# shenyunhang/APE

Measured on AMD Instinct MI355X. Metric: images/sec @1024^2 APE-L_D fwd, higher is better.
Workload: dtype bf16

## Files before the change

### ape_amd/_lib.py

```python
import ctypes
import os
from ctypes import POINTER, Structure, c_char_p, c_double, c_float, c_int, c_int32, c_int64, c_void_p

_HERE = os.path.dirname(os.path.abspath(__file__))
LIB_PATH = os.path.join(_HERE, "lib", "libape_hip.so")

DT_F32 = 0
DT_BF16 = 1
DT_F16 = 2
ACT_NONE, ACT_RELU, ACT_GELU, ACT_SWIGLU, ACT_SILU = 0, 1, 2, 3, 4
MASK_NONE, MASK_ZERO_INPUT, MASK_ZERO_OUTPUT = 0, 1, 2


class GemmArgs(Structure):
    _fields_ = [
        ("A", c_void_p), ("W", c_void_p), ("C", c_void_p), ("bias", c_void_p), ("residual", c_void_p),
        ("rowmask", c_void_p), ("rope_cos", c_void_p), ("rope_sin", c_void_p),
        ("M", c_int32), ("N", c_int32), ("K", c_int32),
        ("lda", c_int32), ("ldw", c_int32), ("ldc", c_int32), ("ldr", c_int32),
        ("in_dt", c_int32), ("out_dt", c_int32), ("res_dt", c_int32),
        ("act", c_int32), ("mask_mode", c_int32), ("trans_out", c_int32),
        ("rope_rows", c_int32), ("rope_hd", c_int32), ("rope_cols", c_int32), ("vec_ok", c_int32),
        ("alpha", c_float), ("clamp", c_float),
        ("splitk", c_int32), ("tile64", c_int32), ("workspace", c_void_p),
# ... 36 lines not shown
    "ape_hip_stuff_collapse": (c_int, [c_void_p, c_int, c_int, c_int, c_int, c_void_p, c_int, c_void_p]),
    "ape_hip_sem_class_weights": (c_int, [c_void_p, c_int, c_void_p, c_void_p, c_int, c_int, c_int, c_float, c_void_p, c_int, c_int, c_void_p]),
    "ape_hip_pan_class_scores": (c_int, [c_void_p, c_int, c_void_p, c_void_p, c_int, c_int, c_float, c_int, c_float, c_void_p, c_void_p,
                                         c_void_p, c_void_p, c_void_p]),
    "ape_hip_argmax_labels": (c_int, [c_void_p, ctypes.c_size_t, c_int, ctypes.c_size_t, c_float, c_void_p, c_void_p]),
    "ape_hip_sdma_usable": (c_int, [c_void_p, c_void_p]),
    "ape_hip_sdma_d2h": (c_int, [c_void_p, c_void_p, ctypes.c_size_t]),
    "ape_hip_sdma_d2h_multi": (c_int, [c_int, ctypes.POINTER(c_void_p), ctypes.POINTER(c_void_p), ctypes.POINTER(ctypes.c_size_t), c_int]),
    "ape_hip_sdma_engines": (c_int, [c_void_p, c_void_p]),
    "ape_hip_row_stats": (c_int, [c_void_p, c_int, c_int, c_int, c_int, c_float, c_void_p, c_void_p, c_void_p]),
    "ape_hip_gemv": (c_int, [c_void_p, c_int, c_void_p, c_int, c_int, c_void_p, c_void_p, c_int, c_int, c_int, c_int,
                             c_float, c_void_p]),
    "ape_hip_gemv_affine": (c_int, [c_void_p, c_int, c_void_p, c_int, c_int, c_void_p, c_void_p, c_int, c_int, c_int, c_int,
                                    c_float, c_void_p, c_void_p, c_int, c_void_p, c_int, c_void_p]),
    "ape_hip_layernorm": (c_int, [POINTER(LayerNormArgs), c_void_p]),
    "ape_hip_postnorm_residual": (c_int, [c_void_p, c_int, c_int, c_void_p, c_void_p, c_float, c_void_p, c_int, c_void_p, c_int, c_int,
                                          c_int, c_int, c_void_p]),
    "ape_hip_groupnorm_workspace_floats": (c_int, [c_int, c_int]),
    "ape_hip_groupnorm": (c_int, [POINTER(GroupNormArgs), c_void_p]),
    "ape_hip_ms_deform_attn_forward": (c_int, [c_void_p, c_int, POINTER(c_int64), POINTER(c_int64), c_void_p, c_void_p,
                                               c_void_p, c_int, c_int, c_int, c_int, c_int, c_int, c_void_p]),
    "ape_hip_msda_fused": (c_int, [c_void_p, c_int, c_int, POINTER(c_int64), POINTER(c_int64), c_void_p, c_int, c_void_p,
                                   c_int, c_void_p, c_int, c_int, c_int, c_int, c_int, c_int, c_void_p]),
    "ape_hip_msda_fused_h": (c_int, [c_void_p, c_int, c_int, POINTER(c_int64), POINTER(c_int64), c_void_p, c_int, c_void_p,
                                     c_int, c_void_p, c_int, c_int, c_int, c_int, c_int, c_int, c_void_p]),
    "ape_hip_attention": (c_int, [c_void_p, c_int, c_void_p, c_int, c_void_p, c_int, c_void_p, c_int, c_int, c_int, c_int,
                                  c_int, c_float, c_int, c_void_p]),
    "ape_hip_geometry": (c_int, [c_int, c_int, c_int, c_int, POINTER(c_int), c_void_p, c_int, c_void_p, c_float, c_float, c_float,
                                 c_void_p, c_int, c_void_p, c_void_p, c_void_p, c_void_p, c_void_p, c_void_p, c_void_p, c_void_p,
                                 c_void_p]),
# ... 5 lines not shown
                                         c_int, c_int, c_float, c_int, c_void_p]),
    "ape_hip_embed_tokens": (c_int, [c_void_p, c_int, c_void_p, c_int, c_void_p, c_int, c_int, c_void_p, c_int, c_int, c_int, c_int,
                                     c_int, c_int, c_void_p]),
    "ape_hip_patchify": (c_int, [c_void_p, c_int, c_int, c_void_p, c_int, c_int, POINTER(c_float), POINTER(c_float), c_void_p,
                                 c_int, c_int, c_void_p]),
    "ape_hip_im2col3x3": (c_int, [c_void_p, c_int, c_void_p, c_int, c_int, c_int, c_void_p, c_int, c_int, c_void_p]),
    "ape_hip_maxpool2x2": (c_int, [c_void_p, c_int, c_void_p, c_int, c_int, c_int, c_void_p, c_int, c_int, c_void_p]),
    "ape_hip_gather_rows": (c_int, [c_void_p, c_int, c_void_p, c_int, c_int, c_void_p, c_int, c_int, c_void_p]),
    "ape_hip_gather_rows_i64": (c_int, [c_void_p, c_int, c_void_p, c_int, c_int, c_void_p, c_int, c_int, c_void_p]),
    "ape_hip_nms_mask_words": (c_int, [c_int]),
    "ape_hip_nms_mask": (c_int, [c_void_p, c_void_p, c_int, c_float, c_void_p, c_void_p]),
    "ape_hip_nms_scan_segments": (c_int, [c_void_p, c_int, c_void_p, c_int, c_int, c_void_p, c_void_p, c_void_p]),
    "ape_hip_nms_scan_classes": (c_int, [c_void_p, c_int, c_void_p, c_int, c_void_p, c_void_p, c_void_p]),
    "ape_hip_vl_pool_workspace_floats": (c_int, [c_int, c_int]),
    "ape_hip_vl_pool": (c_int, [c_void_p, c_int, c_void_p, c_int, c_int, c_int, c_int, c_void_p, c_void_p, c_void_p, c_void_p]),
    "ape_hip_segment_softmax": (c_int, [c_void_p, c_int, c_int, c_int, c_int, c_void_p, c_void_p, c_int, c_int, c_void_p]),
    "ape_hip_colstats_workspace_floats": (c_int, [c_int, c_int]),
    "ape_hip_colstats": (c_int, [c_void_p, c_int, c_int, c_int, c_void_p, c_void_p, c_void_p, c_void_p, c_void_p]),
    "ape_hip_transpose": (c_int, [c_void_p, c_int, c_int, c_int, c_int, c_void_p, c_void_p, c_void_p, c_void_p, c_int, c_int,
                                  c_void_p]),
    "ape_hip_mask_upsample_bits": (c_int, [c_void_p, c_int, c_int, c_int, c_int, c_int, c_int, c_void_p, c_void_p]),
    "ape_hip_roi_align_bits": (c_int, [c_void_p, c_int, c_int, c_void_p, c_int, c_int, c_void_p, c_void_p]),
    "ape_hip_paste_bits": (c_int, [c_void_p, c_int, c_void_p, c_int, c_int, c_int, c_void_p, c_void_p]),
    "ape_hip_mask_upsample_sigmoid": (c_int, [c_void_p, c_int, c_int, c_int, c_int, c_int, c_int, c_int, c_int, c_void_p, c_int, c_int,
                                              c_void_p]),
    "ape_hip_box_refine": (c_int, [c_void_p, c_int, c_void_p, c_void_p, c_int, c_int, c_float, c_void_p, c_void_p, c_void_p]),
    "ape_hip_det_records": (c_int, [c_void_p, c_void_p, c_void_p, c_void_p, c_void_p, c_int, c_void_p, c_void_p, c_void_p, c_void_p]),
    "ape_hip_query_init": (c_int, [c_void_p, c_void_p, c_int, c_void_p, c_int, c_float, c_int, c_void_p, c_void_p, c_int, c_int, c_void_p,
                                   c_void_p]),
    "ape_hip_query_finish": (c_int, [c_void_p, c_int, c_void_p, c_int, c_int, c_int, c_void_p, c_void_p, c_float, c_void_p, c_void_p,
# ... 81 lines not shown
```

### ape_amd/csrc/norm.hip

```cpp
#include "common.h"
#include "../../include/ape_hip.h"

__device__ __forceinline__ float ln_act(float x, int act) {
  if (act == APE_ACT_RELU) return fmaxf(x, 0.f);
  if (act == APE_ACT_GELU) return 0.5f * x * (1.f + erff(x * 0.70710678118654752440f));
  return x;
}

template <typename TX, typename TY, typename TA, int NV4>
__global__ __launch_bounds__(256) void layernorm_kernel(const ApeLayerNormArgs p) {
  const int lane = threadIdx.x & 63;
  const int row = blockIdx.x * 4 + (threadIdx.x >> 6);
  if (row >= p.M) return;
  const TX* x = reinterpret_cast<const TX*>(p.x) + (size_t)row * p.ldx;
  TY* y = reinterpret_cast<TY*>(p.y) + (size_t)row * p.ldy;
  const TA* add = p.add ? reinterpret_cast<const TA*>(p.add) + (size_t)row * p.ldadd : nullptr;
  TY* y2 = p.y2 ? reinterpret_cast<TY*>(p.y2) + (size_t)row * p.ldy2 : nullptr;
  const int C = p.C;
  const float invC = 1.f / (float)C;
  float v[NV4][4];
  float s = 0.f;
#pragma unroll
  for (int i = 0; i < NV4; ++i) {
    const int c = (i * 64 + lane) * 4;
    if (c + 3 < C) {
      ld4<TX>(x + c, v[i]);
    } else {
#pragma unroll
      for (int r = 0; r < 4; ++r) v[i][r] = (c + r < C) ? ldf<TX>(x + c + r) : 0.f;
    }
    s += (v[i][0] + v[i][1]) + (v[i][2] + v[i][3]);
  }
  const float mean = wave_sum(s) * invC;
  float q = 0.f;
#pragma unroll
  for (int i = 0; i < NV4; ++i) {
    const int c = (i * 64 + lane) * 4;
#pragma unroll
    for (int r = 0; r < 4; ++r) {
      const float d = (c + r < C) ? v[i][r] - mean : 0.f;
      q = fmaf(d, d, q);
    }
  }
  const float rstd = rsqrtf(wave_sum(q) * invC + p.eps);
#pragma unroll
  for (int i = 0; i < NV4; ++i) {
    const int c = (i * 64 + lane) * 4;
    if (c >= p.Cpad) continue;
    float o[4], o2[4];
    if (c + 3 < C) {
      float w4[4], b4[4];
      ld4<float>(p.w + c, w4);
      ld4<float>(p.b + c, b4);
#pragma unroll
      for (int r = 0; r < 4; ++r) o[r] = ln_act((v[i][r] - mean) * rstd * w4[r] + b4[r], p.act);
      st4<TY>(y + c, o);
      if (y2 != nullptr) {
        ld4<TA>(add + c, o2);
#pragma unroll
        for (int r = 0; r < 4; ++r) o2[r] += o[r];
        st4<TY>(y2 + c, o2);
      }
      continue;
    }
#pragma unroll
    for (int r = 0; r < 4; ++r) {
      if (c + r < C) {
        o[r] = ln_act((v[i][r] - mean) * rstd * p.w[c + r] + p.b[c + r], p.act);
        o2[r] = (y2 != nullptr) ? o[r] + ldf<TA>(add + c + r) : 0.f;
      } else {
        o[r] = 0.f; o2[r] = 0.f;
      }
    }
    if (c + 3 < p.Cpad) {
      st4<TY>(y + c, o);
      if (y2 != nullptr) st4<TY>(y2 + c, o2);
    } else {
      for (int r = 0; r < 4 && c + r < p.Cpad; ++r) { stf<TY>(y + c + r, o[r]); if (y2 != nullptr) stf<TY>(y2 + c + r, o2[r]); }
    }
  }
  for (int c = NV4 * 256 + lane; c < p.Cpad; c += 64) { stf<TY>(y + c, 0.f); if (y2 != nullptr) stf<TY>(y2 + c, 0.f); }
}

template <typename TX, typename TY, typename TA>
__global__ __launch_bounds__(256) void layernorm_generic_kernel(const ApeLayerNormArgs p) {
  const int lane = threadIdx.x & 63;
  const int row = blockIdx.x * 4 + (threadIdx.x >> 6);
  if (row >= p.M) return;
  const TX* x = reinterpret_cast<const TX*>(p.x) + (size_t)row * p.ldx;
  TY* y = reinterpret_cast<TY*>(p.y) + (size_t)row * p.ldy;
  const TA* add = p.add ? reinterpret_cast<const TA*>(p.add) + (size_t)row * p.ldadd : nullptr;
  TY* y2 = p.y2 ? reinterpret_cast<TY*>(p.y2) + (size_t)row * p.ldy2 : nullptr;
  const int C = p.C;
  const float invC = 1.f / (float)C;
  float s = 0.f;
  for (int c = lane; c < C; c += 64) s += ldf<TX>(x + c);
// ... 366 lines not shown
```

### ape_amd/csrc/vlpool.hip

```cpp
#include "common.h"
#include "../../include/ape_hip.h"

#define VL_CHUNK 128
#define VL_H 8

__global__ __launch_bounds__(256) void vl_smax_partial_kernel(const float* __restrict__ S, int lds, int T, float* __restrict__ pmax) {
  __shared__ float sh[256];
  const int t = threadIdx.x, h = t & 7;
  const int base = blockIdx.x * VL_CHUNK;
  float m = -INFINITY;
  for (int k = 0; k < VL_CHUNK / 32; ++k) {
    const int tok = base + k * 32 + (t >> 3);
    if (tok < T) m = fmaxf(m, S[(size_t)tok * lds + h]);
  }
  sh[t] = m;
  __syncthreads();
  if (t < VL_H) {
    float a = -INFINITY;
    for (int j = t; j < 256; j += 8) a = fmaxf(a, sh[j]);
    pmax[blockIdx.x * VL_H + t] = a;
  }
}

template <typename TX>
// ... 46 lines not shown
  }
  for (int c = t; c < C; c += 256) {
    float acc[VL_H];
#pragma unroll
    for (int h = 0; h < VL_H; ++h) acc[h] = 0.f;
    for (int r = 0; r < cnt; ++r) {
      const float xv = ldf<TX>(x + (size_t)(base + r) * ldx + c);
#pragma unroll
      for (int h = 0; h < VL_H; ++h) acc[h] = fmaf(P[r][h], xv, acc[h]);
    }
#pragma unroll
    for (int h = 0; h < VL_H; ++h) pacc[((size_t)blockIdx.x * VL_H + h) * C + c] = acc[h];
  }
}

__global__ __launch_bounds__(256) void vl_pool_final_kernel(const float* __restrict__ pacc, const float* __restrict__ psum, int nchunk,
                                                            int C, const float* __restrict__ sub, float* __restrict__ out) {
  __shared__ float sa[8][32];
  __shared__ float sl[256];
  const int h = blockIdx.x, t = threadIdx.x;
  const int kg = t >> 5, cl = t & 31;
  const int c = blockIdx.y * 32 + cl;
  float l = 0.f;
  for (int k = t; k < nchunk; k += 256) l += psum[k * VL_H + h];
  sl[t] = l;
  float a = 0.f;
  if (c < C) for (int k = kg; k < nchunk; k += 8) a += pacc[((size_t)k * VL_H + h) * C + c];
  sa[kg][cl] = a;
  __syncthreads();
  for (int o = 128; o > 0; o >>= 1) { if (t < o) sl[t] += sl[t + o]; __syncthreads(); }
  if (t < 32 && c < C) {
    float acc = 0.f;
#pragma unroll
    for (int g = 0; g < 8; ++g) acc += sa[g][t];
    out[h * C + c] = acc / sl[0] - (sub != nullptr ? sub[c] : 0.f);
  }
}

extern "C" int ape_hip_vl_pool_workspace_floats(int T, int C) {
  const int nchunk = ceil_div(T, VL_CHUNK);
  return nchunk * VL_H * (C + 2);
}

extern "C" int ape_hip_vl_pool(const float* S, int lds, const void* x, int ldx, int x_dt, int T, int C, float* workspace,
                               const float* sub, float* out, void* stream) {
  APE_CHECK_ARG(S && x && workspace && out && T > 0 && C > 0, "ape_hip_vl_pool: bad args");
  const int nchunk = ceil_div(T, VL_CHUNK);
  float* pmax = workspace;
  float* psum = pmax + nchunk * VL_H;
  float* pacc = psum + nchunk * VL_H;
  hipStream_t s = (hipStream_t)stream;
  APE_LAUNCH(vl_smax_partial_kernel, dim3(nchunk), dim3(256), 0, s, S, lds, T, pmax);
  if (x_dt == APE_DT_F16) APE_LAUNCH(vl_pool_partial_kernel<f16_t>, dim3(nchunk), dim3(256), 0, s, S, lds, (const f16_t*)x, ldx, T, C, pmax, nchunk, pacc, psum);
  else if (x_dt == APE_DT_BF16) APE_LAUNCH(vl_pool_partial_kernel<bf16_t>, dim3(nchunk), dim3(256), 0, s, S, lds, (const bf16_t*)x, ldx, T, C, pmax, nchunk, pacc, psum);
  else
    APE_LAUNCH(vl_pool_partial_kernel<float>, dim3(nchunk), dim3(256), 0, s, S, lds, (const float*)x, ldx, T, C, pmax, nchunk, pacc, psum);
  APE_LAUNCH(vl_pool_final_kernel, dim3(VL_H, ceil_div(C, 32)), dim3(256), 0, s, pacc, psum, nchunk, C, sub, out);
  APE_CHECK_LAUNCH("ape_hip_vl_pool");
  return 0;
}


template <typename TC>
__global__ __launch_bounds__(256) void head_gemv_kernel(const float* __restrict__ x, int ldx, const float* __restrict__ W,
                                                        const float* __restrict__ bias, float* __restrict__ out, int ldo, int H,
                                                        int N, int D, float alpha, TC* __restrict__ out_bf16, int ldob) {
  const int lane = threadIdx.x & 63;
  const int row = blockIdx.x * 4 + (threadIdx.x >> 6);
  if (row >= H * N) return;
  const int h = row / N, n = row % N;
  const float* w = W + (size_t)row * D;
  const float* xr = x + (size_t)h * ldx;
  float s = 0.f;
// ... 31 lines not shown
```

### ape_amd/layers/fuse_helper.py

```python
import torch
import torch.nn as nn

from .. import ops
from ..packing import attach_cache, f32, ln_params, pack_matrix


class BiMultiHeadAttention(nn.Module):
    def __init__(self, v_dim, l_dim, embed_dim, num_heads, dropout=0.1, stable_softmax_2d=False,
                 clamp_min_for_underflow=True, clamp_max_for_overflow=True, use_attention_mask_v=False):
        super().__init__()
        self.embed_dim, self.num_heads, self.head_dim = embed_dim, num_heads, embed_dim // num_heads
        self.v_dim, self.l_dim = v_dim, l_dim
        assert self.head_dim * num_heads == embed_dim
        self.scale = self.head_dim ** (-0.5)
        self.dropout = dropout
        self.v_proj = nn.Linear(v_dim, embed_dim)
        self.l_proj = nn.Linear(l_dim, embed_dim)
        self.values_v_proj = nn.Linear(v_dim, embed_dim)
        self.values_l_proj = nn.Linear(l_dim, embed_dim)
        self.out_v_proj = nn.Linear(embed_dim, v_dim)
        self.out_l_proj = nn.Linear(embed_dim, l_dim)
        self.stable_softmax_2d = stable_softmax_2d
        self.clamp_min_for_underflow = clamp_min_for_underflow
        self.clamp_max_for_overflow = clamp_max_for_overflow
# ... 84 lines not shown
    def forward_tokens(self, x, lvl_pos, l, dt, defer_language=False):
        if l.shape[0] == 1:
            v_new, qp, ljob = self.forward_tokens_single(x, lvl_pos, l, dt)
        else:
            v_new, qp, l_new = self.forward_tokens_dense(x, lvl_pos, l, dt)
            ljob = ops._Joined(l_new)
        return (v_new, qp, ljob) if defer_language else (v_new, qp, ljob.join())

    def forward_tokens_single(self, x, lvl_pos, l, dt):
        P = self.packed(dt)
        a = self.attn
        l_n = ops.layernorm(l, P["lnl"][0], P["lnl"][1], P["lnl"][2], out_dtype=torch.float32)
        k = ops.gemv(l_n, P["wl"], P["bl"])
        vl = ops.gemv(l_n, P["wvl"], P["bvl"])
        gdv, lnb = ops.gemv(vl, P["wov"], P["bov"], scale=P["gv"], add=P["lnv"][1][None, :])
        v_new, qp = ops.layernorm(x, P["lnv"][0], lnb[0], P["lnv"][2], out_dtype=dt, add=lvl_pos)

        def language_side():
            kh = k.view(a.num_heads, a.head_dim)
            u, u_c = ops.head_gemv(kh, P["wvT"], bf16_copy=dt if dt in ops.HALF16 else True)
            c = ops.head_gemv(kh, P["bv1"], alpha=a.scale)
            _, sbias = ops.gemv(gdv, u, alpha=-a.scale, add=c.view(1, -1))
            S = ops.gemm(v_new, u_c if dt in ops.HALF16 else u, sbias[0], alpha=a.scale, out_dtype=torch.float32)
            pooled = ops.vl_pool(S, v_new, gdv[0])
            ol = ops.head_gemv(pooled, P["wvv"], P["bvv"])
            return ops.gemv(ol.view(1, -1), P["wol"], P["bol"], scale=P["gl"], add=l_n)[1]

        return v_new, qp, ops.fork(language_side)

    def forward(self, v, l, attention_mask_v=None, attention_mask_l=None):
        if attention_mask_l is not None:
            raise NotImplementedError("ape_amd BiAttentionBlock: per-token language masks (un-reduced expression tokens, "
                                      "text_feature_reduce_before_fusion=False) are not implemented")
        dt = getattr(self, "compute_dtype", torch.bfloat16)
        vs, ls = [], []
        for b in range(v.shape[0]):
            zeros = torch.zeros_like(v[b], dtype=dt)
            vn, _, ln = self.forward_tokens(v[b].to(dt).contiguous(), zeros, l[b].float().contiguous(), dt)
            vs.append(vn.to(v.dtype))
# ... 3 lines not shown
```

### ape_amd/ops.py

```python
import ctypes
import math
import os

import numpy as np
import torch

from . import _lib
from ._lib import (ACT_GELU, ACT_NONE, ACT_RELU, ACT_SILU, ACT_SWIGLU, DT_BF16, DT_F32, MASK_NONE,
                   MASK_ZERO_INPUT, MASK_ZERO_OUTPUT)

_DT = {torch.float32: DT_F32, torch.bfloat16: DT_BF16, torch.float16: _lib.DT_F16}
HALF16 = (torch.bfloat16, torch.float16)


def _dt(t):
    try:
        return _DT[t.dtype]
    except KeyError:
        raise TypeError(f"ape_amd: unsupported dtype {t.dtype} (float32 / bfloat16 / float16 only)")


def _dev(*ts):
    for t in ts:
        if t is not None and not t.is_cuda:
# ... 232 lines not shown
        out = torch.empty((M, cpad), dtype=odt, device=x.device)
    args = _lib.LayerNormArgs()
    args.x, args.w, args.b, args.y = x.data_ptr(), _f32vec(w, "w").data_ptr(), _f32vec(b, "b").data_ptr(), out.data_ptr()
    args.M, args.C, args.Cpad = M, C, cpad
    args.ldx, args.ldy = _ld(x), _ld(out)
    args.x_dt, args.y_dt, args.act, args.eps = _dt(x), _dt(out), act, float(eps)
    if add is not None:
        _rowmajor(add, "add")
        if out2 is None:
            out2 = torch.empty((M, cpad), dtype=out.dtype, device=x.device)
        args.add, args.y2, args.ldadd, args.ldy2, args.add_dt = add.data_ptr(), out2.data_ptr(), _ld(add), _ld(out2), _dt(add)
    _lib.check(_lib.load().ape_hip_layernorm(ctypes.byref(args), _stream()), "ape_hip_layernorm")
    return (out, out2) if add is not None else out


def postnorm_residual(stream, t, norm, copy_dtype=None):
    _dev(stream, t)
    _rowmajor(stream, "stream")
    if stream.dtype != torch.float32:
        raise TypeError("ape_amd.ops.postnorm_residual: the residual stream is float32")
    M, C = stream.shape
    if copy_dtype not in (None, torch.float32) + HALF16 or (t is not None and t.dtype not in (torch.float32,) + HALF16):
        raise TypeError("ape_amd.ops.postnorm_residual: t and the copy are float32, bfloat16 or float16")
    copy = torch.empty((M, C), dtype=copy_dtype, device=stream.device) if copy_dtype is not None else None
    w = b = None
    eps = 0.0
    if t is not None:
        _rowmajor(t, "t")
        if tuple(t.shape) != (M, C):
            raise ValueError("ape_amd.ops.postnorm_residual: t must match the stream")
# ... 282 lines not shown


def vl_pool(scores, x, sub=None):
    _dev(scores, x, sub)
    _rowmajor(scores, "scores"), _rowmajor(x, "x")
    if scores.dtype != torch.float32 or scores.shape[1] != 8:
        raise ValueError("ape_amd.ops.vl_pool: scores must be float32 [T,8]")
    T, C = x.shape
    if sub is not None and sub.numel() != C:
        raise ValueError("ape_amd.ops.vl_pool: sub must have one entry per channel")
    lib = _lib.load()
    ws = torch.empty((lib.ape_hip_vl_pool_workspace_floats(T, C),), dtype=torch.float32, device=x.device)
    out = torch.empty((8, C), dtype=torch.float32, device=x.device)
    rc = lib.ape_hip_vl_pool(_p(scores), _ld(scores), _p(x), _ld(x), _dt(x), T, C, _p(ws), _p(_f32vec(sub, "sub")), _p(out), _stream())
    _lib.check(rc, "ape_hip_vl_pool")
    return out


def segment_softmax(scores, nseg, gmax, out_dtype):
    _dev(scores, gmax)
    _rowmajor(scores, "scores")
    if scores.dtype != torch.float32 or gmax.dtype != torch.float32 or scores.shape[1] % nseg:
        raise ValueError("ape_amd.ops.segment_softmax: scores must be float32 [T, nseg*L], gmax a float32 scalar")
    T, C = scores.shape
    out = torch.empty((T, C), dtype=out_dtype, device=scores.device)
    rc = _lib.load().ape_hip_segment_softmax(_p(scores), _ld(scores), T, nseg, C // nseg, _p(gmax), _p(out), _ld(out), _dt(out),
                                             _stream())
    _lib.check(rc, "ape_hip_segment_softmax")
    return out

# ... 962 lines not shown
```

### include/ape_hip.h

```cpp
#ifndef APE_HIP_H
#define APE_HIP_H
#include <stdint.h>

#ifdef __cplusplus
extern "C" {
#endif

#define APE_DT_F32 0
#define APE_DT_BF16 1
#define APE_DT_F16 2

#define APE_ACT_NONE 0
#define APE_ACT_RELU 1
#define APE_ACT_GELU 2
#define APE_ACT_SWIGLU 3
#define APE_ACT_SILU 4

#define APE_MASK_NONE 0
#define APE_MASK_ZERO_INPUT 1
#define APE_MASK_ZERO_OUTPUT 2

const char* ape_hip_last_error(void);
int ape_hip_abi_version(void);
int ape_hip_sizeof_args(int which);
// ... 57 lines not shown

typedef struct ApeLayerNormArgs {
  const void* x;
  const float* w;
  const float* b;
  void* y;
  const void* add;
  void* y2;
  int32_t M, C, Cpad;
  int32_t ldx, ldy, ldadd, ldy2;
  int32_t x_dt, y_dt, add_dt;
  int32_t act;
  float eps;
} ApeLayerNormArgs;
int ape_hip_layernorm(const ApeLayerNormArgs* args, void* stream);

int ape_hip_postnorm_residual(const void* t, int ldt, int t_dt, const float* w, const float* b, float eps, float* stream, int lds,
                              void* copy, int ldc, int copy_dt, int M, int C, void* hip_stream);


typedef struct ApeGroupNormArgs {
  const void* x;
  const float* w;
  const float* b;
  void* y;
  const void* add;
  float* workspace;
  int32_t HW, C, G;
  int32_t ldx, ldy, ldadd;
  int32_t x_dt, y_dt, add_dt;
// ... 27 lines not shown
int ape_hip_im2col3x3(const void* x, int ldx, const int32_t* perm, int H, int W, int C, void* out, int ldo, int dt, void* stream);
int ape_hip_maxpool2x2(const void* x, int ldx, const int32_t* perm, int H, int W, int C, void* out, int ldo, int dt, void* stream);
int ape_hip_gather_rows(const void* x, int ldx, const int32_t* idx, int n, int C, void* out, int ldo, int dt, void* stream);
int ape_hip_gather_rows_i64(const void* x, int ldx, const int64_t* idx, int n, int C, void* out, int ldo, int dt, void* stream);

int ape_hip_nms_mask_words(int n);
int ape_hip_nms_mask(const float* boxes_xyxy, const int32_t* groups, int n, float iou_thr, uint64_t* mask, void* stream);
int ape_hip_nms_scan_segments(const uint64_t* mask, int n, const int32_t* seg_offsets, int num_segments, int max_segment,
                              const uint8_t* valid, uint8_t* keep, void* stream);
int ape_hip_nms_scan_classes(const uint64_t* mask, int n, const int32_t* order, int num_classes, const uint8_t* valid,
                             uint8_t* keep, void* stream);

int ape_hip_vl_pool_workspace_floats(int T, int C);
int ape_hip_vl_pool(const float* S, int lds, const void* x, int ldx, int x_dt, int T, int C, float* workspace, const float* sub,
                    float* out, void* stream);
int ape_hip_head_gemv(const float* x, int ldx, const float* W, const float* bias, float* out, int ldo, int H, int N, int D,
                      float alpha, void* out_bf16, int ldob, int copy_dt, void* stream);

int ape_hip_segment_softmax(const float* S, int lds, int T, int nseg, int L, const float* gmax, void* out, int ldo, int out_dt,
                            void* stream);
int ape_hip_colstats_workspace_floats(int T, int C);
int ape_hip_colstats(const float* S, int lds, int T, int C, const float* gmax, float* workspace, float* colmax, float* colsum,
                     void* stream);
int ape_hip_transpose(const void* S, int lds, int in_dt, int T, int C, const float* gmax, const float* colmax,
                      const float* colsum, void* out, int ldo, int out_dt, void* stream);
int ape_hip_stuff_collapse(const float* logits, int ldl, int Q, int K, int nt, float* out, int ldo, void* stream);
int ape_hip_sem_class_weights(const float* logits, int ldl, const int64_t* qidx, const float* valid_score, int k, int kp, int K, float temp,
                              void* A, int lda, int out_dt, void* stream);
int ape_hip_pan_class_scores(const float* logits, int ldl, const int64_t* qidx, const float* valid_score, int k, int K, float thresh, int transform,
                             float temp, float* score, int64_t* label, int32_t* label32 , uint8_t* keep, void* stream);
// ... 112 lines not shown
```

Before: 115.2.

## Fuse layernorm with VL score projection and per-block maxima, skip separate GEMM

Adds a layernorm_scores kernel that normalizes each 256-wide row, writes both normalized outputs, and immediately dots the result with the 8-head projection u to produce the score matrix S and per-block head maxima. The VL pooling then consumes those precomputed maxima through a new vl_pool_maxima entry and a vectorized partial kernel, dropping the separate score GEMM and the softmax-max pass. Language-side projections are hoisted before the layernorm so the fused kernel has its inputs. This removes two kernel launches and a re-read of v_new, but places a narrow GEMV inside the layernorm and reduces the available overlap with the language side.

```diff
diff --git a/ape_amd/_lib.py b/ape_amd/_lib.py
--- a/ape_amd/_lib.py
+++ b/ape_amd/_lib.py
@@ -74,6 +74,8 @@
     "ape_hip_gemv_affine": (c_int, [c_void_p, c_int, c_void_p, c_int, c_int, c_void_p, c_void_p, c_int, c_int, c_int, c_int,
                                     c_float, c_void_p, c_void_p, c_int, c_void_p, c_int, c_void_p]),
     "ape_hip_layernorm": (c_int, [POINTER(LayerNormArgs), c_void_p]),
+    "ape_hip_layernorm_scores_blocks": (c_int, [c_int]),
+    "ape_hip_layernorm_scores": (c_int, [POINTER(LayerNormArgs), c_void_p, c_int, c_void_p, c_float, c_void_p, c_int, c_void_p, c_void_p]),
     "ape_hip_postnorm_residual": (c_int, [c_void_p, c_int, c_int, c_void_p, c_void_p, c_float, c_void_p, c_int, c_void_p, c_int, c_int,
                                           c_int, c_int, c_void_p]),
     "ape_hip_groupnorm_workspace_floats": (c_int, [c_int, c_int]),
@@ -109,6 +111,8 @@
     "ape_hip_nms_scan_classes": (c_int, [c_void_p, c_int, c_void_p, c_int, c_void_p, c_void_p, c_void_p]),
     "ape_hip_vl_pool_workspace_floats": (c_int, [c_int, c_int]),
     "ape_hip_vl_pool": (c_int, [c_void_p, c_int, c_void_p, c_int, c_int, c_int, c_int, c_void_p, c_void_p, c_void_p, c_void_p]),
+    "ape_hip_vl_pool_maxima": (c_int, [c_void_p, c_int, c_void_p, c_int, c_int, c_int, c_int, c_void_p, c_int, c_void_p, c_void_p, c_void_p,
+                                       c_void_p]),
     "ape_hip_segment_softmax": (c_int, [c_void_p, c_int, c_int, c_int, c_int, c_void_p, c_void_p, c_int, c_int, c_void_p]),
     "ape_hip_colstats_workspace_floats": (c_int, [c_int, c_int]),
     "ape_hip_colstats": (c_int, [c_void_p, c_int, c_int, c_int, c_void_p, c_void_p, c_void_p, c_void_p, c_void_p]),
diff --git a/ape_amd/csrc/norm.hip b/ape_amd/csrc/norm.hip
--- a/ape_amd/csrc/norm.hip
+++ b/ape_amd/csrc/norm.hip
@@ -5,6 +5,87 @@
   if (act == APE_ACT_RELU) return fmaxf(x, 0.f);
   if (act == APE_ACT_GELU) return 0.5f * x * (1.f + erff(x * 0.70710678118654752440f));
   return x;
+}
+
+template <typename TX, int NV4>
+__device__ __forceinline__ float ln_load_row(const TX* x, int C, int lane, float v[NV4][4]) {
+  float s = 0.f;
+#pragma unroll
+  for (int i = 0; i < NV4; ++i) {
+    const int c = (i * 64 + lane) * 4;
+    if (c + 3 < C) {
+      ld4<TX>(x + c, v[i]);
+    } else {
+#pragma unroll
+      for (int r = 0; r < 4; ++r) v[i][r] = (c + r < C) ? ldf<TX>(x + c + r) : 0.f;
+    }
+    s += (v[i][0] + v[i][1]) + (v[i][2] + v[i][3]);
+  }
+  return s;
+}
+
+template <typename TY, typename TA, int NV4, bool KEEP>
+__device__ __forceinline__ void ln_finish_row(const ApeLayerNormArgs& p, float s, const float v[NV4][4], TY* y, const TA* add, TY* y2,
+                                              int lane, float keep[NV4][4]) {
+  const int C = p.C;
+  const float invC = 1.f / (float)C;
+  const float mean = wave_sum(s) * invC;
+  float q = 0.f;
+#pragma unroll
+  for (int i = 0; i < NV4; ++i) {
+    const int c = (i * 64 + lane) * 4;
+#pragma unroll
+    for (int r = 0; r < 4; ++r) {
+      const float d = (c + r < C) ? v[i][r] - mean : 0.f;
+      q = fmaf(d, d, q);
+    }
+  }
+  const float rstd = rsqrtf(wave_sum(q) * invC + p.eps);
+#pragma unroll
+  for (int i = 0; i < NV4; ++i) {
+    const int c = (i * 64 + lane) * 4;
+    if (c >= p.Cpad) continue;
+    float o[4], o2[4];
+    if (c + 3 < C) {
+      float w4[4], b4[4];
+      ld4<float>(p.w + c, w4);
+      ld4<float>(p.b + c, b4);
+#pragma unroll
+      for (int r = 0; r < 4; ++r) o[r] = ln_act((v[i][r] - mean) * rstd * w4[r] + b4[r], p.act);
+      st4<TY>(y + c, o);
+      if (KEEP) {
+#pragma unroll
+        for (int r = 0; r < 4; ++r) keep[i][r] = o[r];
+      }
+      if (y2 != nullptr) {
+        ld4<TA>(add + c, o2);
+#pragma unroll
+        for (int r = 0; r < 4; ++r) o2[r] += o[r];
+        st4<TY>(y2 + c, o2);
+      }
+      continue;
+    }
+#pragma unroll
+    for (int r = 0; r < 4; ++r) {
+      if (c + r < C) {
+        o[r] = ln_act((v[i][r] - mean) * rstd * p.w[c + r] + p.b[c + r], p.act);
+        o2[r] = (y2 != nullptr) ? o[r] + ldf<TA>(add + c + r) : 0.f;
+      } else {
+        o[r] = 0.f; o2[r] = 0.f;
+      }
+    }
+    if (KEEP) {
+#pragma unroll
+      for (int r = 0; r < 4; ++r) keep[i][r] = o[r];
+    }
+    if (c + 3 < p.Cpad) {
+      st4<TY>(y + c, o);
+      if (y2 != nullptr) st4<TY>(y2 + c, o2);
+    } else {
+      for (int r = 0; r < 4 && c + r < p.Cpad; ++r) { stf<TY>(y + c + r, o[r]); if (y2 != nullptr) stf<TY>(y2 + c + r, o2[r]); }
+    }
+  }
+  for (int c = NV4 * 256 + lane; c < p.Cpad; c += 64) { stf<TY>(y + c, 0.f); if (y2 != nullptr) stf<TY>(y2 + c, 0.f); }
 }
 
 template <typename TX, typename TY, typename TA, int NV4>
@@ -16,70 +97,100 @@
   TY* y = reinterpret_cast<TY*>(p.y) + (size_t)row * p.ldy;
   const TA* add = p.add ? reinterpret_cast<const TA*>(p.add) + (size_t)row * p.ldadd : nullptr;
   TY* y2 = p.y2 ? reinterpret_cast<TY*>(p.y2) + (size_t)row * p.ldy2 : nullptr;
-  const int C = p.C;
-  const float invC = 1.f / (float)C;
   float v[NV4][4];
-  float s = 0.f;
-#pragma unroll
-  for (int i = 0; i < NV4; ++i) {
-    const int c = (i * 64 + lane) * 4;
-    if (c + 3 < C) {
-      ld4<TX>(x + c, v[i]);
-    } else {
-#pragma unroll
-      for (int r = 0; r < 4; ++r) v[i][r] = (c + r < C) ? ldf<TX>(x + c + r) : 0.f;
-    }
-    s += (v[i][0] + v[i][1]) + (v[i][2] + v[i][3]);
-  }
-  const float mean = wave_sum(s) * invC;
-  float q = 0.f;
-#pragma unroll
-  for (int i = 0; i < NV4; ++i) {
-    const int c = (i * 64 + lane) * 4;
-#pragma unroll
-    for (int r = 0; r < 4; ++r) {
-      const float d = (c + r < C) ? v[i][r] - mean : 0.f;
-      q = fmaf(d, d, q);
-    }
-  }
-  const float rstd = rsqrtf(wave_sum(q) * invC + p.eps);
-#pragma unroll
-  for (int i = 0; i < NV4; ++i) {
-    const int c = (i * 64 + lane) * 4;
-    if (c >= p.Cpad) continue;
-    float o[4], o2[4];
-    if (c + 3 < C) {
-      float w4[4], b4[4];
-      ld4<float>(p.w + c, w4);
-      ld4<float>(p.b + c, b4);
-#pragma unroll
-      for (int r = 0; r < 4; ++r) o[r] = ln_act((v[i][r] - mean) * rstd * w4[r] + b4[r], p.act);
-      st4<TY>(y + c, o);
-      if (y2 != nullptr) {
-        ld4<TA>(add + c, o2);
-#pragma unroll
-        for (int r = 0; r < 4; ++r) o2[r] += o[r];
-        st4<TY>(y2 + c, o2);
-      }
-      continue;
-    }
-#pragma unroll
-    for (int r = 0; r < 4; ++r) {
-      if (c + r < C) {
-        o[r] = ln_act((v[i][r] - mean) * rstd * p.w[c + r] + p.b[c + r], p.act);
-        o2[r] = (y2 != nullptr) ? o[r] + ldf<TA>(add + c + r) : 0.f;
-      } else {
-        o[r] = 0.f; o2[r] = 0.f;
-      }
-    }
-    if (c + 3 < p.Cpad) {
-      st4<TY>(y + c, o);
-      if (y2 != nullptr) st4<TY>(y2 + c, o2);
-    } else {
-      for (int r = 0; r < 4 && c + r < p.Cpad; ++r) { stf<TY>(y + c + r, o[r]); if (y2 != nullptr) stf<TY>(y2 + c + r, o2[r]); }
-    }
-  }
-  for (int c = NV4 * 256 + lane; c < p.Cpad; c += 64) { stf<TY>(y + c, 0.f); if (y2 != nullptr) stf<TY>(y2 + c, 0.f); }
+  const float s = ln_load_row<TX, NV4>(x, p.C, lane, v);
+  ln_finish_row<TY, TA, NV4, false>(p, s, v, y, add, y2, lane, nullptr);
+}
+
+#define LNS_THREADS 1024
+#define LNS_WAVES (LNS_THREADS / 64)
+#define LNS_MAX_BLOCKS 512
+
+template <typename H>
+__global__ __launch_bounds__(LNS_THREADS) void layernorm_scores_kernel(const ApeLayerNormArgs p_, const H* __restrict__ u, int ldu,
+                                                                       const float* __restrict__ sbias, float alpha,
+                                                                       float* __restrict__ S, int lds, float* __restrict__ pmax) {
+  __shared__ float smax[LNS_WAVES][8];
+  ApeLayerNormArgs p = p_;
+  p.C = 256; p.Cpad = 256; p.act = APE_ACT_NONE;
+  const int lane = threadIdx.x & 63, wave = threadIdx.x >> 6;
+  const int nw = gridDim.x * LNS_WAVES;
+  const int hh = lane >> 3;
+  uint32_t uw[8][2];
+#pragma unroll
+  for (int h = 0; h < 8; ++h) {
+    const uint2 t = *reinterpret_cast<const uint2*>(u + (size_t)h * ldu + lane * 4);
+    uw[h][0] = t.x; uw[h][1] = t.y;
+  }
+  const float sb = sbias[hh];
+  const H* xb = reinterpret_cast<const H*>(p.x);
+  float m = -INFINITY;
+  float v[1][4], vn[1][4];
+  float s = 0.f, sn = 0.f;
+  int row = blockIdx.x * LNS_WAVES + wave;
+  if (row < p.M) s = ln_load_row<H, 1>(xb + (size_t)row * p.ldx, 256, lane, v);
+  for (; row < p.M; row += nw) {
+    if (row + nw < p.M) sn = ln_load_row<H, 1>(xb + (size_t)(row + nw) * p.ldx, 256, lane, vn);
+    float o[1][4];
+    ln_finish_row<H, H, 1, true>(p, s, v, reinterpret_cast<H*>(p.y) + (size_t)row * p.ldy,
+                                 reinterpret_cast<const H*>(p.add) + (size_t)row * p.ldadd,
+                                 reinterpret_cast<H*>(p.y2) + (size_t)row * p.ldy2, lane, o);
+    const uint32_t y0 = h16<H>::pack2(o[0][0], o[0][1]), y1 = h16<H>::pack2(o[0][2], o[0][3]);
+    float d[8];
+#pragma unroll
+    for (int h = 0; h < 8; ++h) d[h] = dot2acc<H>(y1, uw[h][1], dot2acc<H>(y0, uw[h][0], 0.f));
+    float e[4], f[2];
+    {
+      const bool up = (lane & 32) != 0;
+#pragma unroll
+      for (int j = 0; j < 4; ++j) e[j] = (up ? d[j + 4] : d[j]) + __shfl_xor(up ? d[j] : d[j + 4], 32, 64);
+    }
+    {
+      const bool up = (lane & 16) != 0;
+#pragma unroll
+      for (int j = 0; j < 2; ++j) f[j] = (up ? e[j + 2] : e[j]) + __shfl_xor(up ? e[j] : e[j + 2], 16, 64);
+    }
+    const bool up = (lane & 8) != 0;
+    float g = (up ? f[1] : f[0]) + __shfl_xor(up ? f[0] : f[1], 8, 64);
+    g += __shfl_xor(g, 4, 64);
+    g += __shfl_xor(g, 2, 64);
+    g += __shfl_xor(g, 1, 64);
+    const float r = g * alpha + sb;
+    if ((lane & 7) == 0) S[(size_t)row * lds + hh] = r;
+    m = fmaxf(m, r);
+#pragma unroll
+    for (int k = 0; k < 4; ++k) v[0][k] = vn[0][k];
+    s = sn;
+  }
+  if ((lane & 7) == 0) smax[wave][hh] = m;
+  __syncthreads();
+  if (threadIdx.x < 8) {
+    float a = smax[0][threadIdx.x];
+#pragma unroll
+    for (int w = 1; w < LNS_WAVES; ++w) a = fmaxf(a, smax[w][threadIdx.x]);
+    pmax[blockIdx.x * 8 + threadIdx.x] = a;
+  }
+}
+
+extern "C" int ape_hip_layernorm_scores_blocks(int M) { return M <= 0 ? 0 : (ceil_div(M, LNS_WAVES) < LNS_MAX_BLOCKS ? ceil_div(M, LNS_WAVES) : LNS_MAX_BLOCKS); }
+
+extern "C" int ape_hip_layernorm_scores(const ApeLayerNormArgs* a, const void* u, int ldu, const float* sbias, float alpha, float* S,
+                                        int lds, float* pmax, void* stream) {
+  APE_CHECK_ARG(a && a->x && a->y && a->w && a->b && a->add && a->y2 && u && sbias && S && pmax, "ape_hip_layernorm_scores: null pointer");
+  const ApeLayerNormArgs p = *a;
+  APE_CHECK_ARG(p.M > 0 && p.C == 256 && p.Cpad == 256 && p.act == APE_ACT_NONE && lds >= 8 && ldu >= 256,
+                "ape_hip_layernorm_scores: C == Cpad == 256, 8 heads, no activation");
+  APE_CHECK_ARG(ape_is16(p.x_dt) && p.y_dt == p.x_dt && p.add_dt == p.x_dt, "ape_hip_layernorm_scores: x, y, add and u share ONE 16-bit type");
+  APE_CHECK_ARG(p.ldx % 4 == 0 && p.ldy % 4 == 0 && p.ldadd % 4 == 0 && p.ldy2 % 4 == 0 && ldu % 4 == 0 && ((uintptr_t)p.x) % 8 == 0 &&
+                    ((uintptr_t)p.y) % 8 == 0 && ((uintptr_t)p.add) % 8 == 0 && ((uintptr_t)p.y2) % 8 == 0 && ((uintptr_t)u) % 8 == 0 &&
+                    ((uintptr_t)p.w) % 16 == 0 && ((uintptr_t)p.b) % 16 == 0,
+                "ape_hip_layernorm_scores: rows must be 8-byte aligned (ld %% 4 == 0), w / b 16-byte aligned");
+  const dim3 grid(ape_hip_layernorm_scores_blocks(p.M)), block(LNS_THREADS);
+  hipStream_t s = (hipStream_t)stream;
+  if (p.x_dt == APE_DT_F16) APE_LAUNCH(layernorm_scores_kernel<f16_t>, grid, block, 0, s, p, (const f16_t*)u, ldu, sbias, alpha, S, lds, pmax);
+  else APE_LAUNCH(layernorm_scores_kernel<bf16_t>, grid, block, 0, s, p, (const bf16_t*)u, ldu, sbias, alpha, S, lds, pmax);
+  APE_CHECK_LAUNCH("ape_hip_layernorm_scores");
+  return 0;
 }
 
 template <typename TX, typename TY, typename TA>
diff --git a/ape_amd/csrc/vlpool.hip b/ape_amd/csrc/vlpool.hip
--- a/ape_amd/csrc/vlpool.hip
+++ b/ape_amd/csrc/vlpool.hip
@@ -84,49 +84,201 @@
   }
 }
 
+template <typename TX>
+__global__ __launch_bounds__(256) void vl_pool_partial_vec_kernel(const float* __restrict__ S, int lds, const TX* __restrict__ x, int ldx,
+                                                                  int T, int C, const float* __restrict__ pmax, int npmax,
+                                                                  float* __restrict__ pacc, float* __restrict__ psum) {
+  __shared__ __attribute__((aligned(16))) float P[VL_CHUNK][VL_H];
+  __shared__ __attribute__((aligned(16))) float red[4][VL_H * 256];
+  __shared__ float wred[4][VL_H];
+  __shared__ float hmax[VL_H];
+  const int t = threadIdx.x, lane = t & 63, wave = t >> 6;
+  {
+    float4 a = make_float4(-INFINITY, -INFINITY, -INFINITY, -INFINITY);
+    const float4* pm = reinterpret_cast<const float4*>(pmax);
+    for (int j = t; j < npmax * 2; j += 256) {
+      const float4 b = pm[j];
+      a.x = fmaxf(a.x, b.x); a.y = fmaxf(a.y, b.y); a.z = fmaxf(a.z, b.z); a.w = fmaxf(a.w, b.w);
+    }
+#pragma unroll
+    for (int o = 2; o < 64; o <<= 1) {
+      a.x = fmaxf(a.x, __shfl_xor(a.x, o, 64)); a.y = fmaxf(a.y, __shfl_xor(a.y, o, 64));
+      a.z = fmaxf(a.z, __shfl_xor(a.z, o, 64)); a.w = fmaxf(a.w, __shfl_xor(a.w, o, 64));
+    }
+    if (lane < 2) {
+      wred[wave][lane * 4 + 0] = a.x; wred[wave][lane * 4 + 1] = a.y; wred[wave][lane * 4 + 2] = a.z; wred[wave][lane * 4 + 3] = a.w;
+    }
+    __syncthreads();
+    if (t < VL_H) hmax[t] = fmaxf(fmaxf(wred[0][t], wred[1][t]), fmaxf(wred[2][t], wred[3][t]));
+    __syncthreads();
+  }
+  const int base = blockIdx.x * VL_CHUNK;
+  const int cnt = min(VL_CHUNK, T - base);
+  {
+    float g = hmax[0];
+#pragma unroll
+    for (int h = 1; h < VL_H; ++h) g = fmaxf(g, hmax[h]);
+    const int r = t >> 1, h0 = (t & 1) * 4;
+    float pr[4] = {0.f, 0.f, 0.f, 0.f};
+    if (r < cnt) {
+      const float4 sv = *reinterpret_cast<const float4*>(S + (size_t)(base + r) * lds + h0);
+      const float sa[4] = {sv.x, sv.y, sv.z, sv.w};
+#pragma unroll
+      for (int i = 0; i < 4; ++i) {
+        float a = sa[i] - g;
+        a = fminf(fmaxf(a, -50000.f), 50000.f);
+        const float mh = fminf(fmaxf(hmax[h0 + i] - g, -50000.f), 50000.f);
+        float b = a - mh;
+        b = fminf(fmaxf(b, -50000.f), 50000.f);
+        pr[i] = expf(b);
+      }
+    }
+    *reinterpret_cast<float4*>(&P[r][h0]) = make_float4(pr[0], pr[1], pr[2], pr[3]);
+  }
+  __syncthreads();
+  if (blockIdx.y == 0) {
+    const int h = t & 7, j = (t >> 3) * 4;
+    float z = (P[j][h] + P[j + 1][h]) + (P[j + 2][h] + P[j + 3][h]);
+    z += __shfl_xor(z, 8, 64);
+    z += __shfl_xor(z, 16, 64);
+    z += __shfl_xor(z, 32, 64);
+    if (lane < VL_H) wred[wave][lane] = z;
+  }
+  const int cl = t & 31, rg = t >> 5;
+  const int c0 = blockIdx.y * 256 + cl * 8;
+  const bool colok = c0 < C;
+  float acc[VL_H][8];
+#pragma unroll
+  for (int h = 0; h < VL_H; ++h)
+#pragma unroll
+    for (int e = 0; e < 8; ++e) acc[h][e] = 0.f;
+  const TX* xc = x + (size_t)base * ldx + c0;
+#pragma unroll 1
+  for (int i0 = 0; i0 < VL_CHUNK / 8; i0 += 4) {
+    float xv[4][8];
+#pragma unroll
+    for (int j = 0; j < 4; ++j) {
+      const int r = rg + 8 * (i0 + j);
+      if (r < cnt && colok) {
+        ld8<TX>(xc + (size_t)r * ldx, xv[j]);
+      } else {
+#pragma unroll
+        for (int e = 0; e < 8; ++e) xv[j][e] = 0.f;
+      }
+    }
+#pragma unroll
+    for (int j = 0; j < 4; ++j) {
+      const int r = rg + 8 * (i0 + j);
+      const float4 p0 = *reinterpret_cast<const float4*>(&P[r][0]), p1 = *reinterpret_cast<const float4*>(&P[r][4]);
+      const float pv[VL_H] = {p0.x, p0.y, p0.z, p0.w, p1.x, p1.y, p1.z, p1.w};
+#pragma unroll
+      for (int h = 0; h < VL_H; ++h)
+#pragma unroll
+        for (int e = 0; e < 8; ++e) acc[h][e] = fmaf(pv[h], xv[j][e], acc[h][e]);
+    }
+  }
+#pragma unroll
+  for (int h = 0; h < VL_H; ++h)
+#pragma unroll
+    for (int e = 0; e < 8; ++e) acc[h][e] += __shfl_xor(acc[h][e], 32, 64);
+  if (lane < 32) {
+#pragma unroll
+    for (int h = 0; h < VL_H; ++h) {
+      float* d = &red[wave][h * 256 + lane * 8];
+      *reinterpret_cast<float4*>(d) = make_float4(acc[h][0], acc[h][1], acc[h][2], acc[h][3]);
+      *reinterpret_cast<float4*>(d + 4) = make_float4(acc[h][4], acc[h][5], acc[h][6], acc[h][7]);
+    }
+  }
+  __syncthreads();
+  if (blockIdx.y == 0 && t < VL_H) psum[blockIdx.x * VL_H + t] = (wred[0][t] + wred[1][t]) + (wred[2][t] + wred[3][t]);
+  if (colok) {
+    float o[8];
+#pragma unroll
+    for (int e = 0; e < 8; ++e) {
+      const int k = rg * 256 + cl * 8 + e;
+      o[e] = (red[0][k] + red[1][k]) + (red[2][k] + red[3][k]);
+    }
+    float* d = pacc + ((size_t)blockIdx.x * VL_H + rg) * C + c0;
+    *reinterpret_cast<float4*>(d) = make_float4(o[0], o[1], o[2], o[3]);
+    *reinterpret_cast<float4*>(d + 4) = make_float4(o[4], o[5], o[6], o[7]);
+  }
+}
+
+#define VL_FIN_COLS 16
 __global__ __launch_bounds__(256) void vl_pool_final_kernel(const float* __restrict__ pacc, const float* __restrict__ psum, int nchunk,
                                                             int C, const float* __restrict__ sub, float* __restrict__ out) {
-  __shared__ float sa[8][32];
+  __shared__ float sa[16][VL_FIN_COLS];
   __shared__ float sl[256];
   const int h = blockIdx.x, t = threadIdx.x;
-  const int kg = t >> 5, cl = t & 31;
-  const int c = blockIdx.y * 32 + cl;
+  const int kg = t >> 4, cl = t & 15;
+  const int c = blockIdx.y * VL_FIN_COLS + cl;
   float l = 0.f;
   for (int k = t; k < nchunk; k += 256) l += psum[k * VL_H + h];
   sl[t] = l;
-  float a = 0.f;
-  if (c < C) for (int k = kg; k < nchunk; k += 8) a += pacc[((size_t)k * VL_H + h) * C + c];
-  sa[kg][cl] = a;
-  __syncthreads();
-  for (int o = 128; o > 0; o >>= 1) { if (t < o) sl[t] += sl[t + o]; __syncthreads(); }
-  if (t < 32 && c < C) {
-    float acc = 0.f;
-#pragma unroll
-    for (int g = 0; g < 8; ++g) acc += sa[g][t];
-    out[h * C + c] = acc / sl[0] - (sub != nullptr ? sub[c] : 0.f);
-  }
+  float a[4] = {0.f, 0.f, 0.f, 0.f};
+  if (c < C) {
+    const float* pa = pacc + (size_t)h * C + c;
+    int k = kg;
+    for (; k + 48 < nchunk; k += 64) {
+#pragma unroll
+      for (int i = 0; i < 4; ++i) a[i] += pa[(size_t)(k + 16 * i) * VL_H * C];
+    }
+#pragma unroll
+    for (int i = 0; i < 4; ++i)
+      if (k + 16 * i < nchunk) a[i] += pa[(size_t)(k + 16 * i) * VL_H * C];
+  }
+  sa[kg][cl] = (a[0] + a[1]) + (a[2] + a[3]);
+  __syncthreads();
+  float* saf = &sa[0][0];
+  for (int o = 128; o > 0; o >>= 1) {
+    if (t < o) sl[t] += sl[t + o];
+    if (o >= VL_FIN_COLS && t < o) saf[t] += saf[t + o];
+    __syncthreads();
+  }
+  if (t < VL_FIN_COLS && c < C) out[h * C + c] = sa[0][t] / sl[0] - (sub != nullptr ? sub[c] : 0.f);
 }
 
 extern "C" int ape_hip_vl_pool_workspace_floats(int T, int C) {
   const int nchunk = ceil_div(T, VL_CHUNK);
   return nchunk * VL_H * (C + 2);
+}
+
+static int vl_pool_tail(const float* S, int lds, const void* x, int ldx, int x_dt, int T, int C, const float* pmax, int npmax,
+                        float* workspace, const float* sub, float* out, hipStream_t s) {
+  const int nchunk = ceil_div(T, VL_CHUNK);
+  float* psum = workspace + nchunk * VL_H;
+  float* pacc = psum + nchunk * VL_H;
+  const int xb = x_dt == APE_DT_F32 ? 4 : 2;
+  const bool vec = C % 8 == 0 && ldx % 8 == 0 && ((uintptr_t)x) % 16 == 0 && (ldx * xb) % 16 == 0 && lds % 4 == 0 && ((uintptr_t)S) % 16 == 0 &&
+                   ((uintptr_t)pmax) % 16 == 0 && ((uintptr_t)workspace) % 16 == 0;
+  const dim3 gv(nchunk, ceil_div(C, 256));
+  if (vec && x_dt == APE_DT_F16) APE_LAUNCH(vl_pool_partial_vec_kernel<f16_t>, gv, dim3(256), 0, s, S, lds, (const f16_t*)x, ldx, T, C, pmax, npmax, pacc, psum);
+  else if (vec && x_dt == APE_DT_BF16) APE_LAUNCH(vl_pool_partial_vec_kernel<bf16_t>, gv, dim3(256), 0, s, S, lds, (const bf16_t*)x, ldx, T, C, pmax, npmax, pacc, psum);
+  else if (vec) APE_LAUNCH(vl_pool_partial_vec_kernel<float>, gv, dim3(256), 0, s, S, lds, (const float*)x, ldx, T, C, pmax, npmax, pacc, psum);
+  else if (x_dt == APE_DT_F16) APE_LAUNCH(vl_pool_partial_kernel<f16_t>, dim3(nchunk), dim3(256), 0, s, S, lds, (const f16_t*)x, ldx, T, C, pmax, npmax, pacc, psum);
+  else if (x_dt == APE_DT_BF16) APE_LAUNCH(vl_pool_partial_kernel<bf16_t>, dim3(nchunk), dim3(256), 0, s, S, lds, (const bf16_t*)x, ldx, T, C, pmax, npmax, pacc, psum);
+  else
+    APE_LAUNCH(vl_pool_partial_kernel<float>, dim3(nchunk), dim3(256), 0, s, S, lds, (const float*)x, ldx, T, C, pmax, npmax, pacc, psum);
+  APE_LAUNCH(vl_pool_final_kernel, dim3(VL_H, ceil_div(C, VL_FIN_COLS)), dim3(256), 0, s, pacc, psum, nchunk, C, sub, out);
+  return 0;
 }
 
 extern "C" int ape_hip_vl_pool(const float* S, int lds, const void* x, int ldx, int x_dt, int T, int C, float* workspace,
                                const float* sub, float* out, void* stream) {
   APE_CHECK_ARG(S && x && workspace && out && T > 0 && C > 0, "ape_hip_vl_pool: bad args");
   const int nchunk = ceil_div(T, VL_CHUNK);
-  float* pmax = workspace;
-  float* psum = pmax + nchunk * VL_H;
-  float* pacc = psum + nchunk * VL_H;
   hipStream_t s = (hipStream_t)stream;
-  APE_LAUNCH(vl_smax_partial_kernel, dim3(nchunk), dim3(256), 0, s, S, lds, T, pmax);
-  if (x_dt == APE_DT_F16) APE_LAUNCH(vl_pool_partial_kernel<f16_t>, dim3(nchunk), dim3(256), 0, s, S, lds, (const f16_t*)x, ldx, T, C, pmax, nchunk, pacc, psum);
-  else if (x_dt == APE_DT_BF16) APE_LAUNCH(vl_pool_partial_kernel<bf16_t>, dim3(nchunk), dim3(256), 0, s, S, lds, (const bf16_t*)x, ldx, T, C, pmax, nchunk, pacc, psum);
-  else
-    APE_LAUNCH(vl_pool_partial_kernel<float>, dim3(nchunk), dim3(256), 0, s, S, lds, (const float*)x, ldx, T, C, pmax, nchunk, pacc, psum);
-  APE_LAUNCH(vl_pool_final_kernel, dim3(VL_H, ceil_div(C, 32)), dim3(256), 0, s, pacc, psum, nchunk, C, sub, out);
+  APE_LAUNCH(vl_smax_partial_kernel, dim3(nchunk), dim3(256), 0, s, S, lds, T, workspace);
+  vl_pool_tail(S, lds, x, ldx, x_dt, T, C, workspace, nchunk, workspace, sub, out, s);
   APE_CHECK_LAUNCH("ape_hip_vl_pool");
+  return 0;
+}
+
+extern "C" int ape_hip_vl_pool_maxima(const float* S, int lds, const void* x, int ldx, int x_dt, int T, int C, const float* pmax,
+                                      int npmax, float* workspace, const float* sub, float* out, void* stream) {
+  APE_CHECK_ARG(S && x && pmax && workspace && out && T > 0 && C > 0 && npmax > 0, "ape_hip_vl_pool_maxima: bad args");
+  vl_pool_tail(S, lds, x, ldx, x_dt, T, C, pmax, npmax, workspace, sub, out, (hipStream_t)stream);
+  APE_CHECK_LAUNCH("ape_hip_vl_pool_maxima");
   return 0;
 }
 
diff --git a/ape_amd/layers/fuse_helper.py b/ape_amd/layers/fuse_helper.py
--- a/ape_amd/layers/fuse_helper.py
+++ b/ape_amd/layers/fuse_helper.py
@@ -1,8 +1,13 @@
+import os
+
 import torch
 import torch.nn as nn
 
 from .. import ops
 from ..packing import attach_cache, f32, ln_params, pack_matrix
+
+
+VL_FRONT = os.environ.get("APE_VL_FRONT", "1") != "0"
 
 
 class BiMultiHeadAttention(nn.Module):
@@ -122,15 +127,22 @@
         k = ops.gemv(l_n, P["wl"], P["bl"])
         vl = ops.gemv(l_n, P["wvl"], P["bvl"])
         gdv, lnb = ops.gemv(vl, P["wov"], P["bov"], scale=P["gv"], add=P["lnv"][1][None, :])
-        v_new, qp = ops.layernorm(x, P["lnv"][0], lnb[0], P["lnv"][2], out_dtype=dt, add=lvl_pos)
+        kh = k.view(a.num_heads, a.head_dim)
+        u, u_c = ops.head_gemv(kh, P["wvT"], bf16_copy=dt if dt in ops.HALF16 else True)
+        c = ops.head_gemv(kh, P["bv1"], alpha=a.scale)
+        _, sbias = ops.gemv(gdv, u, alpha=-a.scale, add=c.view(1, -1))
+        fused = VL_FRONT and x.is_cuda and dt in ops.HALF16 and ops.layernorm_scores_fusable(x, lvl_pos, dt)
+        if fused:
+            v_new, qp, S, pmax = ops.layernorm_scores(x, P["lnv"][0], lnb[0], P["lnv"][2], lvl_pos, u_c, sbias[0], a.scale)
+        else:
+            v_new, qp = ops.layernorm(x, P["lnv"][0], lnb[0], P["lnv"][2], out_dtype=dt, add=lvl_pos)
 
         def language_side():
-            kh = k.view(a.num_heads, a.head_dim)
-            u, u_c = ops.head_gemv(kh, P["wvT"], bf16_copy=dt if dt in ops.HALF16 else True)
-            c = ops.head_gemv(kh, P["bv1"], alpha=a.scale)
-            _, sbias = ops.gemv(gdv, u, alpha=-a.scale, add=c.view(1, -1))
-            S = ops.gemm(v_new, u_c if dt in ops.HALF16 else u, sbias[0], alpha=a.scale, out_dtype=torch.float32)
-            pooled = ops.vl_pool(S, v_new, gdv[0])
+            if fused:
+                pooled = ops.vl_pool_maxima(S, pmax, v_new, gdv[0])
+            else:
+                S_ = ops.gemm(v_new, u_c if dt in ops.HALF16 else u, sbias[0], alpha=a.scale, out_dtype=torch.float32)
+                pooled = ops.vl_pool(S_, v_new, gdv[0])
             ol = ops.head_gemv(pooled, P["wvv"], P["bvv"])
             return ops.gemv(ol.view(1, -1), P["wol"], P["bol"], scale=P["gl"], add=l_n)[1]
 
diff --git a/ape_amd/ops.py b/ape_amd/ops.py
--- a/ape_amd/ops.py
+++ b/ape_amd/ops.py
@@ -270,6 +270,35 @@
     return (out, out2) if add is not None else out
 
 
+def layernorm_scores_fusable(x, add, dtype):
+    return (x.is_cuda and dtype in HALF16 and x.dtype == dtype and add.dtype == dtype and x.dim() == 2 and x.shape[1] == 256
+            and add.shape == x.shape and x.stride(1) == 1 and add.stride(1) == 1 and _ld(x) % 4 == 0 and _ld(add) % 4 == 0
+            and x.data_ptr() % 8 == 0 and add.data_ptr() % 8 == 0)
+
+
+def layernorm_scores(x, w, b, eps, add, u, sbias, alpha):
+    _dev(x, w, b, add, u, sbias)
+    _rowmajor(x, "x"), _rowmajor(add, "add"), _rowmajor(u, "u")
+    M, C = x.shape
+    if u.shape != (8, C) or u.dtype != x.dtype or add.shape != x.shape or sbias.numel() != 8:
+        raise ValueError("ape_amd.ops.layernorm_scores: u [8, C] in x's dtype, add like x, sbias [8]")
+    lib = _lib.load()
+    out = torch.empty((M, C), dtype=x.dtype, device=x.device)
+    out2 = torch.empty((M, C), dtype=x.dtype, device=x.device)
+    S = torch.empty((M, 8), dtype=torch.float32, device=x.device)
+    pmax = torch.empty((lib.ape_hip_layernorm_scores_blocks(M), 8), dtype=torch.float32, device=x.device)
+    args = _lib.LayerNormArgs()
+    args.x, args.w, args.b, args.y = x.data_ptr(), _f32vec(w, "w").data_ptr(), _f32vec(b, "b").data_ptr(), out.data_ptr()
+    args.M, args.C, args.Cpad = M, C, C
+    args.ldx, args.ldy = _ld(x), _ld(out)
+    args.x_dt, args.y_dt, args.act, args.eps = _dt(x), _dt(out), ACT_NONE, float(eps)
+    args.add, args.y2, args.ldadd, args.ldy2, args.add_dt = add.data_ptr(), out2.data_ptr(), _ld(add), _ld(out2), _dt(add)
+    rc = lib.ape_hip_layernorm_scores(ctypes.byref(args), _p(u), _ld(u), _p(_f32vec(sbias, "sbias")), float(alpha), _p(S), 8, _p(pmax),
+                                      _stream())
+    _lib.check(rc, "ape_hip_layernorm_scores")
+    return out, out2, S, pmax
+
+
 def postnorm_residual(stream, t, norm, copy_dtype=None):
     _dev(stream, t)
     _rowmajor(stream, "stream")
@@ -582,6 +611,25 @@
     out = torch.empty((8, C), dtype=torch.float32, device=x.device)
     rc = lib.ape_hip_vl_pool(_p(scores), _ld(scores), _p(x), _ld(x), _dt(x), T, C, _p(ws), _p(_f32vec(sub, "sub")), _p(out), _stream())
     _lib.check(rc, "ape_hip_vl_pool")
+    return out
+
+
+def vl_pool_maxima(scores, pmax, x, sub=None):
+    _dev(scores, pmax, x, sub)
+    _rowmajor(scores, "scores"), _rowmajor(x, "x")
+    if scores.dtype != torch.float32 or scores.shape[1] != 8:
+        raise ValueError("ape_amd.ops.vl_pool_maxima: scores must be float32 [T,8]")
+    if pmax.dtype != torch.float32 or pmax.dim() != 2 or pmax.shape[1] != 8 or not pmax.is_contiguous():
+        raise ValueError("ape_amd.ops.vl_pool_maxima: pmax must be contiguous float32 [n,8]")
+    T, C = x.shape
+    if sub is not None and sub.numel() != C:
+        raise ValueError("ape_amd.ops.vl_pool_maxima: sub must have one entry per channel")
+    lib = _lib.load()
+    ws = torch.empty((lib.ape_hip_vl_pool_workspace_floats(T, C),), dtype=torch.float32, device=x.device)
+    out = torch.empty((8, C), dtype=torch.float32, device=x.device)
+    rc = lib.ape_hip_vl_pool_maxima(_p(scores), _ld(scores), _p(x), _ld(x), _dt(x), T, C, _p(pmax), pmax.shape[0], _p(ws),
+                                    _p(_f32vec(sub, "sub")), _p(out), _stream())
+    _lib.check(rc, "ape_hip_vl_pool_maxima")
     return out
 
 
diff --git a/include/ape_hip.h b/include/ape_hip.h
--- a/include/ape_hip.h
+++ b/include/ape_hip.h
@@ -95,6 +95,9 @@
   float eps;
 } ApeLayerNormArgs;
 int ape_hip_layernorm(const ApeLayerNormArgs* args, void* stream);
+int ape_hip_layernorm_scores_blocks(int M);
+int ape_hip_layernorm_scores(const ApeLayerNormArgs* args, const void* u, int ldu, const float* sbias, float alpha, float* S, int lds,
+                             float* pmax, void* stream);
 
 int ape_hip_postnorm_residual(const void* t, int ldt, int t_dt, const float* w, const float* b, float eps, float* stream, int lds,
                               void* copy, int ldc, int copy_dt, int M, int C, void* hip_stream);
@@ -152,6 +155,8 @@
 int ape_hip_vl_pool_workspace_floats(int T, int C);
 int ape_hip_vl_pool(const float* S, int lds, const void* x, int ldx, int x_dt, int T, int C, float* workspace, const float* sub,
                     float* out, void* stream);
+int ape_hip_vl_pool_maxima(const float* S, int lds, const void* x, int ldx, int x_dt, int T, int C, const float* pmax, int npmax,
+                           float* workspace, const float* sub, float* out, void* stream);
 int ape_hip_head_gemv(const float* x, int ldx, const float* W, const float* bias, float* out, int ldo, int H, int N, int D,
                       float alpha, void* out_bf16, int ldob, int copy_dt, void* stream);
 
```

Result: no change. 114.4 (-0.6%).
